# 294coder/Dif-PAN

Measured on AMD Instinct MI355X. Metric: fused megapixels/sec at T=1000, WV3 64x64x8 tiles, higher is better.
Workload: dtype f32-class (f16x2 split); 1 GPU; WV3 pansharpening, batch 64 of 64x64x8 tiles per GPU, T=1000 DDPM p_sample, fp32; tiles_per_gpu=64, tiles_total=64, T=1000, model_evaluations=1000, sampler=ddpm, parallelism=tile-shard x1, launches_per_denoising_step=132

## Files before the change

dif-pan_amd/csrc/conv_variants.h:

```cpp
#pragma once
#include "ddif_plan.h"
#include "kernels_conv.h"

namespace ddif {
namespace {

template <int KS, int S, int U, int CK, int PRO, int VEC, int EPI = 0>
ConvVariant variant_for_cfg(int cfg) {
    ConvVariant v;
    switch (cfg) {
        case 0: v.fn = conv_mfma_kernel<KS, S, U, 8, 16, CK, 4, 1, 1, 1, PRO, VEC, EPI>; v.smem = conv_smem_bytes<KS, S, U, 8, 16, CK, 1, PRO>(); v.th = 8; v.tw = 16; v.nt = 32; break;
        case 2: v.fn = conv_mfma_kernel<KS, S, U, 8, 8, CK, 2, 2, 1, 1, PRO, VEC, EPI>; v.smem = conv_smem_bytes<KS, S, U, 8, 8, CK, 2, PRO>(); v.th = 8; v.tw = 8; v.nt = 64; break;
        default: break;
    }
    if constexpr (KS == 1 && VEC == 1) {
        switch (cfg) {
            case 1: v.fn = conv_mfma_kernel<KS, S, U, 8, 16, CK, 4, 1, 1, 2, PRO, VEC, EPI>; v.smem = conv_smem_bytes<KS, S, U, 8, 16, CK, 2, PRO>(); v.th = 8; v.tw = 16; v.nt = 64; break;
            case 3: v.fn = conv_mfma_kernel<KS, S, U, 8, 16, CK, 4, 1, 1, 4, PRO, VEC, EPI>; v.smem = conv_smem_bytes<KS, S, U, 8, 16, CK, 4, PRO>(); v.th = 8; v.tw = 16; v.nt = 128; break;
            case 4: v.fn = conv_mfma_kernel<KS, S, U, 8, 8, CK, 2, 2, 1, 2, PRO, VEC, EPI>; v.smem = conv_smem_bytes<KS, S, U, 8, 8, CK, 4, PRO>(); v.th = 8; v.tw = 8; v.nt = 128; break;
            default: break;
        }
        if constexpr (CK == 32) {
            switch (cfg) {
                case 12: v.fn = conv_mfma_kernel<KS, S, U, 8, 16, CK, 4, 1, 1, 1, PRO, VEC, EPI, 0, 1>; v.smem = conv_smem_bytes<KS, S, U, 8, 16, CK, 1, PRO, 4, 1>(); v.th = 8; v.tw = 16; v.nt = 32; v.x3 = true; break;
// ... 43 lines not shown
        switch (cfg) {
            case 28: v.fn = conv_mfma_kernel<KS, S, U, 8, 16, CK, 4, 1, 1, 1, PRO, VEC, EPI, 0, 3>; v.smem = conv_smem_bytes<KS, S, U, 8, 16, CK, 1, PRO, 4, 3>(); v.th = 8; v.tw = 16; v.nt = 32; v.x3 = v.f16 = true; break;
            case 29: v.fn = conv_mfma_kernel<KS, S, U, 8, 8, CK, 2, 2, 1, 1, PRO, VEC, EPI, 0, 3>; v.smem = conv_smem_bytes<KS, S, U, 8, 8, CK, 2, PRO, 4, 3>(); v.th = 8; v.tw = 8; v.nt = 64; v.x3 = v.f16 = true; break;
            default: break;
        }
    }
    if constexpr (KS == 3 && S == 1 && U == 0 && VEC == 1) {
        switch (cfg) {
            case 5: v.fn = conv_mfma_kernel<KS, S, U, 16, 16, CK, 8, 1, 1, 1, PRO, VEC, EPI>; v.smem = conv_smem_bytes<KS, S, U, 16, 16, CK, 1, PRO, 8>(); v.th = 16; v.tw = 16; v.nt = 32; v.nthr = 512; break;
            case 6: v.fn = conv_mfma_kernel<KS, S, U, 16, 16, CK, 8, 1, 1, 2, PRO, VEC, EPI>; v.smem = conv_smem_bytes<KS, S, U, 16, 16, CK, 2, PRO, 8>(); v.th = 16; v.tw = 16; v.nt = 64; v.nthr = 512; break;
            default: break;
        }
    }
    return v;
}
template <int KS, int S, int U, int CK, int PRO, int VEC>
ConvVariant variant_small_tiles(int cfg) {
    return (cfg >= 2) ? variant_for_cfg<KS, S, U, CK, PRO, VEC>(cfg) : ConvVariant();
}
}
}
```

dif-pan_amd/csrc/ddif_capi.cpp:

```cpp
#include "ddif_plan.h"

struct ddif_net {
    ddif::Net n;
};
struct ddif_plan {
    ddif::Plan p;
};

namespace ddif {
extern int g_debug_grid_cap;
}

struct DeviceScope {
    int prev = -1;
    bool ok = true;
    explicit DeviceScope(int dev) {
        if (hipGetDevice(&prev) != hipSuccess) prev = -1;
        if (prev != dev) ok = hipSetDevice(dev) == hipSuccess;
    }
    ~DeviceScope() {
        int cur = -1;
        if (prev >= 0 && hipGetDevice(&cur) == hipSuccess && cur != prev) (void)hipSetDevice(prev);
    }
};
#define DDIF_PLAN_ENTER(plan, what)                                                                                   \
    if (!(plan)) return ddif::fail(DDIF_ERR_INVALID, what ": NULL plan");                                             \
    DeviceScope dscope__((plan)->p.net->device);                                                                      \
    if (!dscope__.ok) return ddif::fail(DDIF_ERR_HIP, what ": hipSetDevice(%d) failed", (plan)->p.net->device);      \
    if ((plan)->p.generation != (plan)->p.net->generation)                                                            \
        return ddif::fail(DDIF_ERR_STATE, what ": the network's weights were re-committed after this plan was built " \
                                               "(its launch program points into the old weight blob); create a new plan"); \
    if ((plan)->p.net->merged_stale && !(plan)->p.train_mode)                                                         \
        return ddif::fail(DDIF_ERR_STATE, what ": the weights were refreshed on the device for training (ddif_net_refresh), which leaves the "   \
                                               "inference-only merged FFN weights stale; load + commit the weights again before inference")

#define DDIF_GUARD_BEGIN try {
#define DDIF_GUARD_END                                                                    \
    }                                                                                     \
    catch (const std::exception& e) {                                                     \
        return ddif::fail(DDIF_ERR_INVALID, "unexpected C++ exception: %s", e.what());    \
    }                                                                                     \
    catch (...) {                                                                         \
        return ddif::fail(DDIF_ERR_INVALID, "unexpected C++ exception");                  \
    }

extern "C" {

int ddif_net_create(ddif_net_t* out, const ddif_net_cfg* cfg, int device) {
    DDIF_GUARD_BEGIN
// ... 389 lines not shown
```

dif-pan_amd/csrc/ddif_conv_k3.cpp:

```cpp
#include "conv_variants.h"

namespace ddif {

ConvVariant get_conv_variant_k3(int stride, int ups, int ck, int pro, int cfg, int vec) {
    ConvVariant v;
    const bool plain = stride == 1 && !ups;
    if (ck != 16) return v;
    if (vec == 2) {
        if (plain && pro == PRO_NONE) { v = variant_for_cfg<3, 1, 0, 16, PRO_NONE, 2>(cfg); v.name = "conv3x3_cat"; }
    } else if (!vec) {
        if (plain && pro == PRO_NONE) { v = variant_for_cfg<3, 1, 0, 16, PRO_NONE, 0>(cfg); v.name = "conv3x3_scalar"; }
    } else if (plain && pro == PRO_GN_SILU) { v = variant_for_cfg<3, 1, 0, 16, PRO_GN_SILU, 1>(cfg); v.name = "conv3x3_gn_silu"; }
    else if (plain && pro == PRO_NONE) { v = variant_for_cfg<3, 1, 0, 16, PRO_NONE, 1>(cfg); v.name = "conv3x3"; }
    else if (stride == 2 && !ups && pro == PRO_NONE) { v = variant_small_tiles<3, 2, 0, 16, PRO_NONE, 1>(cfg); v.name = "conv3x3_s2"; }
    else if (stride == 1 && ups && pro == PRO_NONE) { v = variant_for_cfg<3, 1, 1, 16, PRO_NONE, 1>(cfg); v.name = "conv3x3_up2"; }
    return v;
}

}
```

dif-pan_amd/csrc/ddif_net.cpp:

```cpp
#include "ddif_net.h"
#include <cstdint>
#include <tuple>
#include "kernels_refresh.h"

namespace ddif {

thread_local std::string g_err;

int fail(int code, const char* fmt, ...) {
    char buf[1024];
    va_list ap;
    va_start(ap, fmt);
    vsnprintf(buf, sizeof(buf), fmt, ap);
    va_end(ap);
    g_err = buf;
    return code;
}

static bool in_list(const int32_t* a, int n, int v) {
    for (int i = 0; i < n; ++i)
        if (a[i] == v) return true;
    return false;
}

// ... 221 lines not shown
                                for (int pl = 0; pl < 2; ++pl) {
                                    const size_t fl = (((((size_t)nbi * n_chunks + ch) * taps + tap) * K16 + k16) * 2 + pl) * 256 + (size_t)(h * 32 + j) * 4;
                                    o[fl * 2 + t] = q[pl];
                                }
                            }
    return off;
}

size_t pack_conv_b1(Blob& b, size_t x3_off, int cout, int cin, int ks, int ck) {
    const size_t steps = (size_t)((((cout + 31) / 32 + 3) & ~3)) * ((cin + ck - 1) / ck) * (ks * ks) * (ck / 16);
    const size_t off = b.add(nullptr, steps * 256);
    for (size_t st = 0; st < steps; ++st) std::memcpy(b.v.data() + off + st * 256, b.v.data() + x3_off + st * 3 * 256, 256 * sizeof(float));
    return off;
}

}

int Net::commit(hipStream_t stream) {
    Blob b;
    struct PendConv { std::string name; size_t w_off; long bias_off; int cin, cout, ks, ck, n_chunks; long x3_off = -1; long f16_off = -1; long b1_off = -1; };
    std::vector<PendConv> pend;
    std::map<std::string, size_t> vec_off;
    std::string missing;
    recipes.clear();
    auto rec_pack = [&](int kind, const std::string& s0, const std::string& s1, size_t off, int cout, int cin0, int cin1, int ks, int ck, int n_chunks) {
        Recipe r;
        r.kind = kind;
        r.src0 = s0;
        r.src1 = s1;
        r.dst_off = off;
        r.cout = cout;
        r.cin0 = cin0;
        r.cin1 = cin1;
        r.ks = ks;
        r.ck = ck;
// ... 107 lines not shown
                    for (int nb = 0; nb < co / 32; ++nb)
                        for (int ln = 0; ln < 64; ++ln)
                            for (int sx = 0; sx < 16; ++sx)
                                r[((size_t)nb * 64 + ln) * 16 + sx] = wx->v[(size_t)(32 * nb + (ln & 31)) * 32 + 8 * (sx >> 2) + 4 * (ln >> 5) + (sx & 3)];
                    vec_off[L.p + ".cond_inj.x_conv.xf"] = b.add(r.data(), r.size());
                }
            }
        }
    }
    for (auto& L : mid) {
        add_slot(L.p + ".res_block");
        add_resblock(L.p + ".res_block");
        if (L.attn) add_attn(L.p + ".attn");
    }
    for (auto& L : ups) {
        if (L.kind == L_UP) { add_conv(L.p + ".conv", true); continue; }
        add_slot(L.p + ".res_block");
        add_resblock(L.p + ".res_block");
        if (L.attn) add_attn(L.p + ".attn");
        const std::string ci = L.p + ".cond_inj";
        add_vec(ci + ".prenorm_x.weight");
        add_vec(ci + ".prenorm_x.bias");
        add_dw(ci + ".q.0.weight");
        add_conv(ci + ".q.1", true);
        add_dw(ci + ".kv.0.weight");
        add_conv(ci + ".kv.1", true);
        const HostTensor *wo = need(ci + ".attn_out.weight"), *bo = need(ci + ".attn_out.bias");
        const HostTensor* wr = get(ci + ".attn_res.weight");
        const HostTensor* br = get(ci + ".attn_res.bias");
        if (wo) {
            vec_off[ci + ".attn_out.weight"] = b.add(wo->v.data(), wo->v.size());
// ... 121 lines not shown
        blob = nullptr;
    }
    blob_floats = b.v.size() + 64;
    DDIF_HIPCHK(hipMalloc((void**)&blob, blob_floats * sizeof(float)));
    DDIF_HIPCHK(hipMemcpy(blob, b.v.data(), b.v.size() * sizeof(float), hipMemcpyHostToDevice));
    (void)stream;

    conv.clear();
    vec.clear();
    for (auto& p : pend) {
        PackedConv pc;
        pc.w = blob + p.w_off;
        pc.w_x3 = p.x3_off >= 0 ? blob + p.x3_off : nullptr;
        pc.w_f16 = p.f16_off >= 0 ? blob + p.f16_off : nullptr;
        pc.w_b1 = p.b1_off >= 0 ? blob + p.b1_off : nullptr;
        pc.bias = p.bias_off >= 0 ? blob + p.bias_off : nullptr;
        pc.cin = p.cin;
        pc.cout = p.cout;
        pc.ks = p.ks;
        pc.ck = p.ck;
        pc.n_chunks = p.n_chunks;
        conv[p.name] = pc;
    }
    vec_absmax.clear();
    for (auto& kv : vec_off) {
        vec[kv.first] = blob + kv.second;
        float m = 0.f;
        if (const HostTensor* t = get(kv.first))
            for (float x : t->v) m = std::fabs(x) > m || std::isnan(x) ? (std::isnan(x) ? INFINITY : std::fabs(x)) : m;
        vec_absmax[blob + kv.second] = m;
// ... 173 lines not shown
```

dif-pan_amd/csrc/ddif_net.h:

```cpp
#pragma once
#include <mutex>
#include <cmath>
#include <cstdarg>
#include <cstdint>
#include <cstdio>
#include <cstring>
#include <functional>
#include <map>
#include <memory>
#include <string>
#include <vector>

#include "../../include/ddif.h"
#include "../../include/ddif_testops.h"
#include "ddif_dev.h"

namespace ddif {

extern thread_local std::string g_err;
int fail(int code, const char* fmt, ...);

#define DDIF_HIPCHK(x)                                                                                      \
    do {                                                                                                    \
        hipError_t e__ = (x);                                                                               \
// ... 6 lines not shown

enum LayerKind { L_STEM, L_ENC, L_DOWN, L_MID, L_DEC, L_UP };

struct Layer {
    LayerKind kind;
    int cin = 0, cout = 0, cx = 0, cskip = 0;
    bool attn = false;
    std::string p;
};

struct PackedConv {
    const float* w = nullptr;
    const float* w_x3 = nullptr;
    const float* w_f16 = nullptr;
    const float* w_b1 = nullptr;
    const float* bias = nullptr;
    int cin = 0, cout = 0, ks = 1, ck = 32, n_chunks = 0;
};

struct HostTensor {
    std::vector<float> v;
    std::vector<int64_t> shape;
};

struct Net {
    ddif_net_cfg cfg{};
    int device = 0;
    std::vector<Layer> downs, mid, ups;
    int final_in = 0;
    std::map<std::string, HostTensor> host;
// ... 59 lines not shown
```

dif-pan_amd/csrc/ddif_plan.cpp:

```cpp
#include "ddif_plan.h"
#include <algorithm>
#include "kernels_conv.h"
#include "kernels_misc.h"
#include "attn_args.h"
#include "kernels_lafuse.h"

namespace ddif {

ConvVariant get_conv_variant(int ks, int stride, int ups, int ck, int pro, int cfg, int vec, int epi, int math) {
    if (cfg == 20 || cfg == 21)
        return (stride == 1 && !ups && vec == 1) ? get_lr_variant(ks, cfg == 20 ? 2 : 4, pro, epi, (math == MATH_F16X2 && pro == PRO_COLSM) ? MATH_BF16X3 : math) : ConvVariant();
    if (ks == 1) return get_conv_variant_k1(stride, ups, ck, pro, cfg, vec, epi);
    if (ks == 3) return epi ? get_conv_variant_k3e(stride, ups, ck, pro, cfg, vec, epi) : get_conv_variant_k3(stride, ups, ck, pro, cfg, vec);
    return ConvVariant();
}

static int num_cus();
static int x3_enabled() {
    static const int x3 = [] { const char* e = getenv("DDIF_X3"); return e ? atoi(e) : 1; }();
    return x3;
}
static int f16_enabled() {
    static const int f16 = [] { const char* e = getenv("DDIF_F16"); return e ? atoi(e) : 1; }();
    return f16;
}
int g_math_mode = [] { const char* e = getenv("DDIF_MATH"); return (e && std::strcmp(e, "bf16") == 0) ? 1 : 0; }();
int g_f16_raw = [] { const char* e = getenv("DDIF_F16_RAW"); return e ? (atoi(e) != 0) : 1; }();
static int lr_rows_enabled() {
    static const int v = [] { const char* e = getenv("DDIF_LR_ROWS"); return e ? atoi(e) : 1; }();
    return v;
}
static int lafuse_enabled() {
    static const int v = [] { const char* e = getenv("DDIF_LAFUSE"); return e ? atoi(e) : 1; }();
    return v;
}
static int xcd_mask() {
    static const int v = [] { const char* e = getenv("DDIF_XCD"); return e ? atoi(e) : 15; }();
    return v;
}
static int la8_enabled() {
    static const int v = [] { const char* e = getenv("DDIF_LA8"); return e ? atoi(e) : 1; }();
    return v;
}
static int xf_enabled() {
// ... 236 lines not shown
        return fail(DDIF_ERR_INVALID, "%s: a tensor of this batch reaches 4 GiB (32-bit offsets); split the batch", s.name);
    bool f16ok = f16_enabled() && !train_mode && pc.w_f16 && !s.w_override && !s.exact;
    const bool raw_in = !(s.pro == PRO_GN || s.pro == PRO_GN_SILU || s.pro == PRO_GN_DW);
    if (raw_in && !f16_raw) f16ok = false;
    if (f16ok && (s.pro == PRO_GN || s.pro == PRO_GN_SILU)) {
        auto ig = net->vec_absmax.find(s.gamma), ib = net->vec_absmax.find(s.beta);
        const double n = (double)(c0 + c1) * Hin * Win;
        f16ok = ig != net->vec_absmax.end() && ib != net->vec_absmax.end() && std::sqrt(n) * ig->second + ib->second < DDIF_F16_AMAX;
    }
    const bool b1ok = math_mode == 1 && !train_mode && pc.w_b1 && !s.w_override && !s.exact;
    const bool f16ok0 = f16ok;
    if (b1ok) f16ok = false;
    int math = b1ok ? MATH_BF16X1 : (f16ok ? MATH_F16X2 : MATH_BF16X3);
    int cfg = pick_cfg(pc.ks, pc.ck, s.pro, vec, s.stride, s.ups, Hout, Wout, pc.cout, B, c0 + c1, c1 ? c0 : c0 + c1, true, s.exact, f16ok, b1ok);
    const int epi = (s.film ? EPI_FILM : 0) | (s.res ? EPI_RES : 0) | (pc.cout % 4 != 0 ? EPI_SOUT : 0) | (s.silu ? EPI_SILU : 0) | (s.cso_mx ? EPI_COLST : 0);
    if (s.cso_mx && ((cfg != 20 && cfg != 21) || Hout > (cfg == 20 ? 8 : 16)))
        return fail(DDIF_ERR_INVALID, "%s: column statistics epilogue needs the low-resolution kernel and H <= 16", s.name);
    static const bool wres_env = [] { const char* e = getenv("DDIF_WRES"); return !e || atoi(e) != 0; }();
    if (cfg == 27 && wres_env && c0 == 32 && c1 == 0 && pc.cout <= 32 && pc.ck == 16 && pc.n_chunks == 2 && !s.w_override && s.w_bstride == 0 &&
        get_conv_variant(pc.ks, s.stride, s.ups, pc.ck, s.pro, 37, vec, epi, math).fn)
        cfg = 37;
    ConvVariant var = get_conv_variant(pc.ks, s.stride, s.ups, pc.ck, s.pro, cfg, vec, epi, math);
    if (!var.fn && (cfg == 20 || cfg == 21)) {
        cfg = pick_cfg(pc.ks, pc.ck, s.pro, vec, s.stride, s.ups, Hout, Wout, pc.cout, B, c0 + c1, c1 ? c0 : c0 + c1, false, false, f16ok, b1ok);
        var = get_conv_variant(pc.ks, s.stride, s.ups, pc.ck, s.pro, cfg, vec, epi);
    }
    if (!var.fn && b1ok) {
        f16ok = f16ok0;
        math = f16ok ? MATH_F16X2 : MATH_BF16X3;
        cfg = pick_cfg(pc.ks, pc.ck, s.pro, vec, s.stride, s.ups, Hout, Wout, pc.cout, B, c0 + c1, c1 ? c0 : c0 + c1, true, s.exact, f16ok, false);
        var = get_conv_variant(pc.ks, s.stride, s.ups, pc.ck, s.pro, cfg, vec, epi, math);
        if (!var.fn && (cfg == 20 || cfg == 21)) {
            cfg = pick_cfg(pc.ks, pc.ck, s.pro, vec, s.stride, s.ups, Hout, Wout, pc.cout, B, c0 + c1, c1 ? c0 : c0 + c1, false, false, f16ok, false);
            var = get_conv_variant(pc.ks, s.stride, s.ups, pc.ck, s.pro, cfg, vec, epi);
        }
    }
    if (!var.fn) return fail(DDIF_ERR_INVALID, "%s: no kernel variant (ks=%d stride=%d ups=%d ck=%d pro=%d cfg=%d vec=%d epi=%d)", s.name, pc.ks, s.stride, s.ups, pc.ck, s.pro, cfg, vec, epi);
// ... 27 lines not shown
        use(s.cso_mx);
        use(s.cso_sm);
    }
    if (int e = alloc_tensor(out, pc.cout, Hout, Wout, &prog == &step)) return e;
    if (xf) {
        if (int e = alloc_tensor(&s.xf->out, s.xf->pc->cout, Hout, Wout, true)) return e;
    }
    ConvArgs a{};
    a.in0 = s.in0.p;
    a.in1 = s.in1.p;
    a.c0 = c0;
    a.c1 = c1;
    a.B = B;
    a.Hin = Hin;
    a.Win = Win;
    a.Hout = Hout;
    a.Wout = Wout;
    a.Cout = pc.cout;
    a.w = s.w_override ? s.w_override : (var.b1 ? pc.w_b1 : (var.f16 ? pc.w_f16 : (var.x3 ? pc.w_x3 : pc.w)));
    if (var.x3 && !s.w_override && !a.w) return fail(DDIF_ERR_STATE, "%s: split-operand variant without split weights", s.name);
    a.w_bstride = s.w_bstride;
    a.cs_mx = s.cs_mx;
    a.cs_sm = s.cs_sm;
    a.dw_w = s.dw_w;
    a.out_xn = s.out_xn;
    a.cso_mx = s.cso_mx;
    a.cso_sm = s.cso_sm;
    if (s.pro == PRO_GN_DW && (!s.dw_w || c0 + c1 > 256)) return fail(DDIF_ERR_INVALID, "%s: depthwise staging needs weights and <= 256 channels", s.name);
    if (s.pro == PRO_COLSM && (!s.cs_mx || !s.cs_sm || c0 % pc.ck != 0)) return fail(DDIF_ERR_INVALID, "%s: column-softmax prologue needs statistics and c0 %% %d == 0", s.name, pc.ck);
    a.n_chunks = var.wr ? 1 : pc.n_chunks;
    a.bias = (s.use_bias && pc.bias) ? pc.bias : zeros;
    a.tbias = zeros;
    a.st0 = s.in0.st;
    a.np0 = s.in0.np;
    a.st1 = s.in1.st;
    a.np1 = s.in1.np;
    a.gamma = s.gamma;
    a.beta = s.beta;
    a.res = s.res;
    a.film = s.film;
    a.out = out->p;
    a.tiles_x = (Wout + var.tw - 1) / var.tw;
    a.tiles_y = (Hout + var.th - 1) / var.th;
    const int gy = (pc.cout + var.nt - 1) / var.nt;
    const bool st_halves = !var.lr && var.th == 16 && var.tw == 16 && var.nthr == 512;
    a.st_halves = st_halves ? 1 : 0;
    a.tiles_y8 = (Hout + 7) / 8;
    const int np_out = st_halves ? a.tiles_x * a.tiles_y8 : a.tiles_x * a.tiles_y;
    if (s.stats) {
        out->np = np_out * gy;
        if (int e = dalloc(&out->st, (size_t)B * out->np * 2)) return e;
        a.st_out = out->st;
    }
    a.n_ct = gy;
    if (xf) {
        if (gy != 1 || !s.stats) return fail(DDIF_ERR_STATE, "%s: x_conv fold needs one cout tile and output statistics", s.name);
        s.xf->out.np = np_out;
        if (int e = dalloc(&s.xf->out.st, (size_t)B * s.xf->out.np * 2)) return e;
        a.xf_w = s.xf->w;
        a.xf_b = s.xf->pc->bias;
        a.xf_film = s.xf->film;
        a.xf_out = s.xf->out.p;
// ... 31 lines not shown
        const ConvVariant vs = get_conv_variant(pc.ks, s.stride, s.ups, pc.ck, s.pro, cfg, vec, EPI_SAMP, math);
        if (vs.fn && vs.smem == var.smem) {
            fn_samp = vs.fn;
            if (var.smem + 8192 > 64 * 1024)
                DDIF_HIPCHK(hipFuncSetAttribute(reinterpret_cast<const void*>(fn_samp), hipFuncAttributeMaxDynamicSharedMemorySize, (int)(var.smem + 8192)));
            final_fused = true;
        }
    }
    const float* lms_p = lms.p;
    const bool dyn = s.dyn_input;
    const bool self_c = net->cfg.self_condition != 0;
    const int tb_off = s.tb_off;
    static const bool dump = getenv("DDIF_DUMP_PLAN") != nullptr;
    if (dump)
        fprintf(stderr, "[ddif plan] %-34s %-24s ks=%d s=%d u=%d  %3d+%3d -> %3d  @%3dx%-3d pro=%d epi=%d cfg=%d items=%ld grid=%u smem=%zu  in@%p out@%p\n", s.name, var.name, pc.ks, s.stride,
                s.ups, c0, c1, pc.cout, Hout, Wout, s.pro, epi, cfg, nwork, grid.x, smem, (const void*)s.in0.p, (const void*)out->p);
    Op op;
    op.name = var.name;
    {
        char lb[160];
        snprintf(lb, sizeof lb, "%s %dx%d %d+%d->%d @%dx%d cfg%d", s.name, pc.ks, pc.ks, c0, c1, pc.cout, Hout, Wout, cfg);
        op.label = lb;
    }
    op.flop = 2.0 * B * Hout * Wout * (double)pc.cout * (c0 + c1) * pc.ks * pc.ks;
    op.bytes = 4.0 * B * ((double)Hin * Win * (c0 + c1) + (double)Hout * Wout * pc.cout);
    if (xf) {
        op.label += " + x_conv+FiLM";
        op.flop += 2.0 * B * Hout * Wout * 32.0 * s.xf->pc->cout;
        op.bytes += 4.0 * B * (double)Hout * Wout * 3.0 * s.xf->pc->cout;
    }
    op.cls = (Hout * Wout <= 256) ? 2 : (pc.ks == 3 ? 0 : 1);
    op.mfma_w = var.b1 ? 1 : (var.f16 ? 3 : (var.x3 ? 6 : 16));
    op.timed = op.cls == 0;
    if (pc.ks == 3 && &prog == &step) {
        ++n_conv3;
        if (var.x3) ++n_conv3_x3;
        if (var.f16) ++n_conv3_f16;
        if (var.b1) ++n_conv3_b1;
    }
// ... 1527 lines not shown
```

dif-pan_amd/csrc/kernels_conv.h:

```cpp
#pragma once
#include "ddif_dev.h"
#include "sampler_dev.h"

namespace ddif {

struct ConvArgs {
    const float* in0;
    const float* in1;
    int c0, c1;
    int B, Hin, Win;
    int Hout, Wout, Cout;
    const float* w;
    int n_chunks;
    const float* bias;
    const float* tbias;
    int tbias_stride;
    const int* step_ptr;
    int tb_rowstride;
    const double* st0;
    int np0;
    const double* st1;
    int np1;
    const float* gamma;
    const float* beta;
// ... 28 lines not shown
    int xf_cout;
    int st_halves;
    int tiles_y8;
};

template <int F>
struct StageKind {
    static constexpr bool LAST = (F & 1) != 0;
    static constexpr bool TAIL = (F & 2) != 0;
};

enum { EPI_FILM = 1, EPI_SOUT = 2, EPI_RES = 4, EPI_SILU = 8, EPI_TBS = 16, EPI_COLST = 32, EPI_SAMP = 64, EPI_XF1 = 128, EPI_XF2 = 256 };
template <int KS, int STRIDE, int UPS, int TH, int TW, int CK, int WM, int WN, int MB, int NB, int PRO, int VEC, int EPI = 0, int ABL = 0, int MATH = 0>
__global__ __launch_bounds__(64 * WM * WN) void conv_mfma_kernel(ConvArgs a) {
    constexpr int NW = WM * WN, NTHR = 64 * NW;
    constexpr int PAD = KS / 2;
    constexpr int IH = (TH - 1) * STRIDE + KS, IW = (TW - 1) * STRIDE + KS;
    constexpr bool X3 = MATH >= 1;
    constexpr bool F16 = MATH == 3 || MATH == 5;
    constexpr bool WR = MATH == 5;
    constexpr bool B1 = MATH == 4;
    constexpr int NPL = F16 ? 2 : (B1 ? 1 : 3);
    constexpr bool WSB = MATH == 2;
    constexpr int NWB = (WSB || WR) ? 1 : 2;
    constexpr int PS = CK / 2;
    constexpr int LDA = X3 ? NPL * PS + 4 : CK + 4;
    constexpr int LDH = CK + 4;
    constexpr int TAPS = KS * KS;
    constexpr int K8 = CK / 8;
    constexpr int K16 = CK / 16;
    constexpr int C4 = CK / 4;
    constexpr int NF = X3 ? TAPS * K16 : TAPS * K8;
    constexpr int RP = (X3 && KS == 3 && STRIDE == 1) ? (WR ? (64 - (IW * LDA) % 64) % 64 : (NPL == 2 ? 24 : (NPL == 1 ? 40 : 8))) : 0;
    constexpr int LDR = IW * LDA + RP;
    constexpr int ABUF = IH * LDR;
    constexpr bool DWM = (PRO == PRO_GN_DW);
    constexpr bool GNP = (PRO == PRO_GN || PRO == PRO_GN_SILU || PRO == PRO_GN_DW);
    constexpr bool FILM = (EPI & EPI_FILM) != 0, SOUT = (EPI & EPI_SOUT) != 0, RES = (EPI & EPI_RES) != 0, SILU = (EPI & EPI_SILU) != 0, TBS = (EPI & EPI_TBS) != 0;
    constexpr bool SAMP = (EPI & EPI_SAMP) != 0;
    constexpr int NBX = (EPI & EPI_XF1) ? 1 : ((EPI & EPI_XF2) ? 2 : 0);
    constexpr bool XF = NBX > 0;
    static_assert(!SAMP || (!SOUT && !RES && !FILM), "sampler epilogue: the plain vector epilogue of the final conv");
    static_assert(!XF || (MB == 1 && NB == 1 && WN == 1 && !SOUT && !SAMP && !FILM && !SILU && PRO != PRO_GN_DW), "x_conv + FiLM fold: one wave holds all 32 couts of its pixels");
// ... 7 lines not shown
    constexpr int NITEMS = (LH * LW * C4 + NTHR - 1) / NTHR;
    constexpr int WCHUNK = X3 ? NF * NPL * 256 : NF * 256;
    constexpr int WBUF = NB * WN * WCHUNK;
    constexpr int WITEMS = WR ? 0 : (WBUF / 4 + NTHR - 1) / NTHR;
    constexpr int WITEMS_A = WITEMS ? WITEMS : 1;
    constexpr int WRI = WR ? (WBUF / 4 + NTHR - 1) / NTHR : 1;
    constexpr int DUMMY = DWM ? CK : (X3 ? NPL * PS : CK);
    static_assert(NW == 4 || NW == 8, "4 or 8 wavefronts per workgroup");
    static_assert(!X3 || (CK % 16 == 0 && (VEC == 1 || (VEC == 2 && F16 && PRO == PRO_NONE))), "split-operand paths: 16-channel slabs, float4 staging (per-thread source select: the stem on f16x2)");
    static_assert(TH * TW == 32 * MB * WM, "pixel tile must match the wave layout");
    static_assert(CK % 8 == 0 && NTHR % C4 == 0, "chunk size");
    static_assert(NITEMS <= 32, "valid mask is 32 bits");
    static_assert(!F16 || PRO != PRO_COLSM, "f16x2: the column-softmax prologue stays on bf16x3 / fp32 (probabilities far below 2^-7)");
    static_assert(RP == 0 || !DWM, "row pad: 3x3 tiles only");
    static_assert(!WR || (KS == 3 && STRIDE == 1 && !UPS && CK == 32 && TW == 16 && !DWM), "resident weights: plain 3x3 convs with one 32-channel stage");

    dd_touch_kernargs<sizeof(ConvArgs)>();
    DDIF_DYN_SMEM(smem);
    float* As = reinterpret_cast<float*>(smem);
    float* Ws = As + 2 * ABUF;
    double* red = reinterpret_cast<double*>(smem + (size_t)(2 * ABUF + NWB * WBUF) * sizeof(float));
    float* Hs = reinterpret_cast<float*>(smem + (size_t)(2 * ABUF + NWB * WBUF) * sizeof(float) + 4 * NW * sizeof(double));
    float* DWs = Hs + HBUF;
    [[maybe_unused]] double* redx = reinterpret_cast<double*>(DWs + DWMAX);
    float* GBs = DWs + DWMAX + (XF ? 8 * NW : 0);
    float* BTs = GBs + (GNP ? 2 * a.n_chunks * CK : 0);
    [[maybe_unused]] float* BXs = BTs + a.n_ct * (32 * NB * WN);

    const int tid = threadIdx.x, lane = tid & 63;
#ifdef DDIF_EMU
    const int wave = tid >> 6;
    [[maybe_unused]] const long long t_entry = 0;
#else
    const int wave = __builtin_amdgcn_readfirstlane(tid >> 6);
    [[maybe_unused]] const long long t_entry = (ABL & 16) ? (long long)__builtin_amdgcn_s_memtime() : 0;
#endif
    const int wm = wave / WN, wn = wave % WN;
    const int h = lane >> 5, j = lane & 31;
    const int tiles = a.tiles_x * a.tiles_y;
    const int ntiles = a.B * tiles;
    const int nwork = ntiles * a.n_ct;
    int w0, w1;
    wg_work_range(nwork, &w0, &w1, a.xcd);
    if (w0 >= w1) return;
    const int Hc = UPS ? a.Hin * 2 : a.Hin, Wc = UPS ? a.Win * 2 : a.Win;
    const int Ctot = a.c0 + a.c1;
    const int GBN = a.n_chunks * CK;
    const int c4 = tid % C4;
    const int stepv = a.step_ptr ? *a.step_ptr : 0;
    const float* tbrow = a.tbias;
    [[maybe_unused]] SamplerRun s_run{};
    [[maybe_unused]] int s_k = 0;
    [[maybe_unused]] float s_c0 = 0.f, s_c1 = 0.f, s_c2 = 0.f, s_c3 = 0.f, s_c4 = 0.f;
    [[maybe_unused]] const float* s_noise = nullptr;
    if constexpr (SAMP) {
        s_run = *a.s_run;
        s_k = *a.step_ptr;
        s_c0 = s_run.tab[0][s_k];
        s_c1 = s_run.tab[1][s_k];
        s_c2 = s_run.tab[2][s_k];
// ... 2 lines not shown
            s_c4 = s_run.tab[4][s_k];
        }
        s_noise = s_run.noise ? s_run.noise + (size_t)s_k * ((size_t)a.B * a.Cout * a.Hout * a.Wout) : nullptr;
        if (blockIdx.x == 0 && tid == 0) *a.s_step_next = s_k + 1;
    }

    int abase[MB], e_my[MB], e_mx[MB];
    unsigned e_off[MB], e_foff[MB];
    [[maybe_unused]] unsigned e_xoff[MB], e_xfoff[MB];
#pragma unroll
    for (int mb = 0; mb < MB; ++mb) {
        const int m = (wm * MB + mb) * 32 + j;
        abase[mb] = (m / TW) * STRIDE * LDR + (m % TW) * STRIDE * LDA + 4 * h;
        e_my[mb] = m / TW;
        e_mx[mb] = m % TW;
        e_off[mb] = (unsigned)(((e_my[mb] * a.Wout + e_mx[mb]) * a.Cout + 4 * h) * 4);
        e_foff[mb] = (unsigned)(((e_my[mb] * a.Wout + e_mx[mb]) * 2 * a.Cout + 4 * h) * 4);
        if constexpr (XF) {
            e_xoff[mb] = (unsigned)(((e_my[mb] * a.Wout + e_mx[mb]) * (32 * NBX) + 4 * h) * 4);
            e_xfoff[mb] = (unsigned)(((e_my[mb] * a.Wout + e_mx[mb]) * 2 * (32 * NBX) + 4 * h) * 4);
        }
    }
    [[maybe_unused]] float xw[XF ? NBX : 1][16];
    if constexpr (XF) {
#pragma unroll
        for (int nx = 0; nx < NBX; ++nx)
#pragma unroll
            for (int q = 0; q < 4; ++q) {
                const float4 t = *reinterpret_cast<const float4*>(a.xf_w + ((size_t)(nx * 64 + lane) * 16 + 4 * q));
                xw[nx][4 * q + 0] = t.x;
                xw[nx][4 * q + 1] = t.y;
// ... 58 lines not shown
    Pos L = locate(w0);
    int l_ch = 0;
    [[maybe_unused]] int l_sp[(VEC == 1) ? 1 : NITEMS];
    [[maybe_unused]] unsigned l_o0[NITEMS], l_o1[NITEMS];
    unsigned l_cso[PRO == PRO_COLSM ? NITEMS : 1];
    unsigned l_ok = 0;
    auto item_geometry = [&]() {
        const int iy0 = L.oy0 * STRIDE - LPAD, ix0 = L.ox0 * STRIDE - LPAD;
        l_ok = 0;
#pragma unroll
        for (int it = 0; it < NITEMS; ++it) {
            const int iy = iy0 + a_py[it], ix = ix0 + a_px[it];
            const bool ok = (iy >= 0) & (iy < Hc) & (ix >= 0) & (ix < Wc);
            l_ok |= (ok ? 1u : 0u) << it;
            const int iyc = iy < 0 ? 0 : (iy >= Hc ? Hc - 1 : iy), ixc = ix < 0 ? 0 : (ix >= Wc ? Wc - 1 : ix);
            const int sp = (L.b * a.Hin + (UPS ? (iyc >> 1) : iyc)) * a.Win + (UPS ? (ixc >> 1) : ixc);
            if constexpr (VEC == 1) {
                l_o0[it] = (unsigned)sp * (unsigned)(a.c0 * 4);
                if (a.c1) l_o1[it] = (unsigned)sp * (unsigned)(a.c1 * 4);
            } else {
                l_sp[it] = sp;
            }
            if (PRO == PRO_COLSM) l_cso[it] = (unsigned)(L.b * a.Win + ixc) * (unsigned)(a.c0 * 4);
        }
        l_ok &= a_in;
    };

    struct StageRegs {
        float4 sv[NITEMS], wv[WITEMS_A];
        float4 mxv[PRO == PRO_COLSM ? NITEMS : 1], smv[PRO == PRO_COLSM ? NITEMS : 1];
        unsigned ok;
// ... 265 lines not shown
        if ((ABL & 16) && a.dbg && tid == 0 && dbg_n < 126) a.dbg[blockIdx.x * 128 + dbg_n++] = (long long)__builtin_amdgcn_s_memtime();
#endif
    };
#ifndef DDIF_EMU
    if ((ABL & 16) && a.dbg && tid == 0) a.dbg[blockIdx.x * 128 + dbg_n++] = t_entry;
#endif
    f32x16 acc[MB][NB];
    const int nflat = (w1 - w0) * a.n_chunks;

    auto stage = [&](auto kind, const int cur, StageRegs& Rn, StageRegs& Rf) {
        constexpr bool LAST = decltype(kind)::LAST, TAIL = decltype(kind)::TAIL;
        stamp();
        const float* Ac = As + cur * ABUF;
        const Pos Cp = bufpos[cur];
        const int c_ch = bufch[cur];
        const int nbg0 = (Cp.ct * WN + wn) * NB;
        float4 e_t[(LAST && TBS) ? NB : 1][4];
        float4 e_res[(LAST && RES) ? MB : 1][(LAST && RES) ? NB : 1][4];
        float4 e_fs[(LAST && FILM) ? MB : 1][(LAST && FILM) ? NB : 1][4], e_fh[(LAST && FILM) ? MB : 1][(LAST && FILM) ? NB : 1][4];
        [[maybe_unused]] float4 e_xi[(LAST && SAMP) ? MB : 1][(LAST && SAMP) ? NB : 1][4], e_xl[(LAST && SAMP) ? MB : 1][(LAST && SAMP) ? NB : 1][4];
        [[maybe_unused]] float4 e_xs[(LAST && XF) ? NBX : 1][4], e_xh[(LAST && XF) ? NBX : 1][4];
        [[maybe_unused]] unsigned e_pxo = 0;
        bool full = true;
        unsigned e_po[MB], e_pf[MB];
        bool e_pok[MB];
        size_t tile_el = 0;
        if constexpr (LAST) {
            full = (Cp.oy0 + TH <= a.Hout) & (Cp.ox0 + TW <= a.Wout);
            const size_t tile_pix = (size_t)((Cp.b * a.Hout + Cp.oy0) * a.Wout + Cp.ox0);
            tile_el = tile_pix * a.Cout + nbg0 * 32;
#pragma unroll
            for (int mb = 0; mb < MB; ++mb) {
                e_pok[mb] = full || ((Cp.oy0 + e_my[mb] < a.Hout) & (Cp.ox0 + e_mx[mb] < a.Wout));
                e_po[mb] = e_pok[mb] ? e_off[mb] : (unsigned)(16 * h);
                e_pf[mb] = e_pok[mb] ? e_foff[mb] : (unsigned)(16 * h);
            }
            if constexpr (!SOUT) {
                const int nbl = nbg0 * 32 < a.Cout ? nbg0 * 32 : 0;
                [[maybe_unused]] const char* tb = reinterpret_cast<const char*>(tbrow + (size_t)Cp.b * a.tbias_stride + nbl);
                [[maybe_unused]] const char* rbase = reinterpret_cast<const char*>(a.res + tile_pix * a.Cout + nbl);
                [[maybe_unused]] const char* fbase = reinterpret_cast<const char*>(a.film + tile_pix * 2 * a.Cout + nbl);
                [[maybe_unused]] const char* xibase = reinterpret_cast<const char*>(a.s_img + tile_pix * a.Cout + nbl);
                [[maybe_unused]] const char* xlbase = reinterpret_cast<const char*>(a.s_lms + tile_pix * a.Cout + nbl);
#pragma unroll
// ... 35 lines not shown
        if (c_ch == 0) {
#pragma unroll
            for (int mb = 0; mb < MB; ++mb)
#pragma unroll
                for (int nb = 0; nb < NB; ++nb)
#pragma unroll
                    for (int r = 0; r < 16; ++r) acc[mb][nb][r] = 0.f;
        }
        if constexpr (ILV && !TAIL) fs_begin(Rn);
        const float* Wc = Ws + ((WSB || WR) ? 0 : cur) * WBUF + (wn * NB) * WCHUNK + h * 128 + j * 4;
        if constexpr (X3) {
            constexpr int FB = (MB * NB >= 2) ? 1 : 2;
            float4 xa[FB][MB][NPL], wb[FB][NB][NPL];
            auto load_frags3 = [&](int f, int slot) {
                const int tap = WR ? f % TAPS : f / K16, k16 = WR ? f / TAPS : f % K16;
                const int aoff = (tap / KS) * LDR + (tap % KS) * LDA + k16 * 8;
#pragma unroll
                for (int q = 0; q < NPL; ++q) {
#pragma unroll
                    for (int mb = 0; mb < MB; ++mb)
                        xa[slot][mb][q] = (ABL & 128) ? make_float4(1.f, 2.f, 3.f, (float)(f + q)) : *reinterpret_cast<const float4*>(&Ac[abase[mb] + aoff + q * PS]);
#pragma unroll
                    for (int nb = 0; nb < NB; ++nb)
                        wb[slot][nb][q] = (ABL & 128) ? make_float4(4.f, 3.f, 2.f, (float)(f - q)) : *reinterpret_cast<const float4*>(&Wc[nb * WCHUNK + (f * NPL + q) * 256]);
                }
            };
            if (FB == 2) load_frags3(0, 0);
#pragma unroll
            for (int tap = 0; tap < NF; ++tap) {
                if (FB == 2) {
                    if (tap + 1 < NF) load_frags3(tap + 1, (tap + 1) & 1);
// ... 285 lines not shown
    if (DWM) {
#pragma unroll
        for (int k = 0; k < DWI; ++k) {
            const int i = tid + k * NTHR;
            if (i < 9 * Ctot) DWs[i] = t_dw[k];
        }
    }
    if (GNP) {
        gn_reduce_partials(gp, a.st0, a.np0, a.st1, a.np1, R0.pos.b, (double)Ctot * a.Hin * a.Win, &mean, &rstd);
        gn_b = R0.pos.b;
    }
    __syncthreads();
    stamp();
    finish_stage(R0, 0);
    {
        const int nbt = a.n_ct * (32 * NB * WN);
#pragma unroll
        for (int k = 0; k < TBL; ++k) {
            const int i = tid + k * NTHR;
            if (i < nbt) BTs[i] = t_bias[k] + t_tb[k];
        }
        for (int i = tid + TBL * NTHR; i < nbt; i += NTHR) {
            const int c = i < a.Cout ? i : a.Cout - 1;
            BTs[i] = a.bias[c] + (TBS ? 0.f : tbrow[c]);
        }
        if constexpr (XF) {
            if (tid < 32 * NBX) BXs[tid] = a.xf_b[tid];
        }
    }
    __syncthreads();
    stamp();
// ... 15 lines not shown
    if (nflat & 1) stage(StageKind<3>{}, 0, R1, R0);
    __syncthreads();
    flush_stats();
    stamp();
    if constexpr (RANGE) {
        if (a.range_flag && !(r_max < 65520.f)) *a.range_flag = 1;
    }
}


template <int KS, int STRIDE, int UPS, int TH, int TW, int CK, int NBT, int PRO = 0, int NW = 4, int MATH = 0>
constexpr size_t conv_smem_bytes() {
    constexpr int IH = (TH - 1) * STRIDE + KS, IW = (TW - 1) * STRIDE + KS;
    constexpr size_t dw = PRO == PRO_GN_DW ? (size_t)((TH + 2) * (TW + 2) * (CK + 4) + 9 * 256) : 0;
    constexpr int npl = (MATH == 3 || MATH == 5) ? 2 : (MATH == 4 ? 1 : 3);
    constexpr int lda = MATH >= 1 ? npl * CK / 2 + 4 : CK + 4, wchunk = MATH >= 1 ? KS * KS * (CK / 16) * npl * 256 : KS * KS * (CK / 8) * 256;
    constexpr int rp = (MATH >= 1 && KS == 3 && STRIDE == 1) ? (MATH == 5 ? (64 - (IW * lda) % 64) % 64 : (npl == 2 ? 24 : (npl == 1 ? 40 : 8))) : 0;
    return (size_t)(2 * IH * (IW * lda + rp) + ((MATH == 2 || MATH == 5) ? 1 : 2) * NBT * wchunk + dw) * sizeof(float) + 4 * NW * sizeof(double);
}
inline size_t conv_smem_extra(int pro, int n_chunks, int ck, int cout_pad, int xf_cout = 0) {
    return ((pro == PRO_GN || pro == PRO_GN_SILU || pro == PRO_GN_DW) ? (size_t)2 * n_chunks * ck : 0) * sizeof(float) + (size_t)cout_pad * sizeof(float) +
           (xf_cout ? (size_t)xf_cout * sizeof(float) + 32 * sizeof(double) : 0);
}

}
```

Baseline: 0.07824 MP/s.

## Fold nearest-upsample into 3x3 conv as four 2x2 polyphase convs

Nearest-2x upsample followed by a 3x3 conv is rewritten as four phase-specific 2x2 convolutions on the low-resolution input. The weights are pre-summed on the host at commit time into a 4*cout f16x2 pack. The kernel gains a polyphase mode that selects the phase from the output-channel tile, offsets the input window, and writes interleaved outputs. This cuts the MACs from 9 to 4 taps per output and avoids reading the upsampled input. In exchange it adds a new kernel variant, a larger grid, and a separate weight pack that goes stale after weight refresh.

```diff
diff --git a/dif-pan_amd/csrc/conv_variants.h b/dif-pan_amd/csrc/conv_variants.h
--- a/dif-pan_amd/csrc/conv_variants.h
+++ b/dif-pan_amd/csrc/conv_variants.h
@@ -81,6 +81,16 @@
     }
     return v;
 }
+inline ConvVariant variant_up_poly(int cfg) {
+    ConvVariant v;
+    switch (cfg) {
+        case 27: v.fn = conv_mfma_kernel<3, 1, 2, 16, 16, 16, 8, 1, 1, 2, PRO_NONE, 1, 0, 0, 3>; v.smem = conv_smem_bytes<3, 1, 2, 16, 16, 16, 2, PRO_NONE, 8, 3>(); v.th = 16; v.tw = 16; v.nt = 64; v.nthr = 512; v.x3 = v.f16 = true; break;
+        case 28: v.fn = conv_mfma_kernel<3, 1, 2, 8, 16, 16, 4, 1, 1, 2, PRO_NONE, 1, 0, 0, 3>; v.smem = conv_smem_bytes<3, 1, 2, 8, 16, 16, 2, PRO_NONE, 4, 3>(); v.th = 8; v.tw = 16; v.nt = 64; v.x3 = v.f16 = true; break;
+        case 29: v.fn = conv_mfma_kernel<3, 1, 2, 8, 8, 16, 2, 2, 1, 1, PRO_NONE, 1, 0, 0, 3>; v.smem = conv_smem_bytes<3, 1, 2, 8, 8, 16, 2, PRO_NONE, 4, 3>(); v.th = 8; v.tw = 8; v.nt = 64; v.x3 = v.f16 = true; break;
+        default: break;
+    }
+    return v;
+}
 template <int KS, int S, int U, int CK, int PRO, int VEC>
 ConvVariant variant_small_tiles(int cfg) {
     return (cfg >= 2) ? variant_for_cfg<KS, S, U, CK, PRO, VEC>(cfg) : ConvVariant();
diff --git a/dif-pan_amd/csrc/ddif_capi.cpp b/dif-pan_amd/csrc/ddif_capi.cpp
--- a/dif-pan_amd/csrc/ddif_capi.cpp
+++ b/dif-pan_amd/csrc/ddif_capi.cpp
@@ -32,7 +32,7 @@
                                                "(its launch program points into the old weight blob); create a new plan"); \
     if ((plan)->p.net->merged_stale && !(plan)->p.train_mode)                                                         \
         return ddif::fail(DDIF_ERR_STATE, what ": the weights were refreshed on the device for training (ddif_net_refresh), which leaves the "   \
-                                               "inference-only merged FFN weights stale; load + commit the weights again before inference")
+                                               "inference-only packs (merged FFN weights, f16x2 planes, polyphase Upsample folds) stale; load + commit the weights again before inference")
 
 #define DDIF_GUARD_BEGIN try {
 #define DDIF_GUARD_END                                                                    \
diff --git a/dif-pan_amd/csrc/ddif_conv_k3.cpp b/dif-pan_amd/csrc/ddif_conv_k3.cpp
--- a/dif-pan_amd/csrc/ddif_conv_k3.cpp
+++ b/dif-pan_amd/csrc/ddif_conv_k3.cpp
@@ -13,7 +13,8 @@
     } else if (plain && pro == PRO_GN_SILU) { v = variant_for_cfg<3, 1, 0, 16, PRO_GN_SILU, 1>(cfg); v.name = "conv3x3_gn_silu"; }
     else if (plain && pro == PRO_NONE) { v = variant_for_cfg<3, 1, 0, 16, PRO_NONE, 1>(cfg); v.name = "conv3x3"; }
     else if (stride == 2 && !ups && pro == PRO_NONE) { v = variant_small_tiles<3, 2, 0, 16, PRO_NONE, 1>(cfg); v.name = "conv3x3_s2"; }
-    else if (stride == 1 && ups && pro == PRO_NONE) { v = variant_for_cfg<3, 1, 1, 16, PRO_NONE, 1>(cfg); v.name = "conv3x3_up2"; }
+    else if (stride == 1 && ups == 1 && pro == PRO_NONE) { v = variant_for_cfg<3, 1, 1, 16, PRO_NONE, 1>(cfg); v.name = "conv3x3_up2"; }
+    else if (stride == 1 && ups == 2 && pro == PRO_NONE) { v = variant_up_poly(cfg); v.name = "conv3x3_up2_poly"; }
     return v;
 }
 
diff --git a/dif-pan_amd/csrc/ddif_net.cpp b/dif-pan_amd/csrc/ddif_net.cpp
--- a/dif-pan_amd/csrc/ddif_net.cpp
+++ b/dif-pan_amd/csrc/ddif_net.cpp
@@ -259,11 +259,27 @@
     return off;
 }
 
+std::vector<float> fold_up_poly(const float* w, int cout, int cin) {
+    static const int lo[2][2] = {{0, 1}, {0, 2}}, hi[2][2] = {{0, 2}, {1, 2}};
+    std::vector<float> f((size_t)4 * cout * cin * 4);
+    for (int ph = 0; ph < 4; ++ph)
+        for (int o = 0; o < cout; ++o)
+            for (int i = 0; i < cin; ++i)
+                for (int t = 0; t < 4; ++t) {
+                    const int py = ph >> 1, px = ph & 1, ty = t >> 1, tx = t & 1;
+                    double acc = 0.0;
+                    for (int ky = lo[py][ty]; ky <= hi[py][ty]; ++ky)
+                        for (int kx = lo[px][tx]; kx <= hi[px][tx]; ++kx) acc += (double)w[((size_t)o * cin + i) * 9 + ky * 3 + kx];
+                    f[(((size_t)ph * cout + o) * cin + i) * 4 + t] = (float)acc;
+                }
+    return f;
+}
+
 }
 
 int Net::commit(hipStream_t stream) {
     Blob b;
-    struct PendConv { std::string name; size_t w_off; long bias_off; int cin, cout, ks, ck, n_chunks; long x3_off = -1; long f16_off = -1; long b1_off = -1; };
+    struct PendConv { std::string name; size_t w_off; long bias_off; int cin, cout, ks, ck, n_chunks; long x3_off = -1; long f16_off = -1; long b1_off = -1; long up4_off = -1; };
     std::vector<PendConv> pend;
     std::map<std::string, size_t> vec_off;
     std::string missing;
@@ -401,7 +417,17 @@
         if (L.attn) add_attn(L.p + ".attn");
     }
     for (auto& L : ups) {
-        if (L.kind == L_UP) { add_conv(L.p + ".conv", true); continue; }
+        if (L.kind == L_UP) {
+            add_conv(L.p + ".conv", true);
+            const HostTensor* w = get(L.p + ".conv.weight");
+            if (w && w->shape.size() == 4 && w->shape[2] == 3 && w->shape[3] == 3 && !pend.empty() && pend.back().name == L.p + ".conv") {
+                const int co = (int)w->shape[0], cin = (int)w->shape[1];
+                const std::vector<float> f = fold_up_poly(w->v.data(), co, cin);
+                const size_t off = pack_conv_f16(b, f.data(), 4 * co, cin, 2, 16);
+                pend.back().up4_off = off == (size_t)-1 ? -1 : (long)off;
+            }
+            continue;
+        }
         add_slot(L.p + ".res_block");
         add_resblock(L.p + ".res_block");
         if (L.attn) add_attn(L.p + ".attn");
@@ -553,6 +579,7 @@
         pc.w_x3 = p.x3_off >= 0 ? blob + p.x3_off : nullptr;
         pc.w_f16 = p.f16_off >= 0 ? blob + p.f16_off : nullptr;
         pc.w_b1 = p.b1_off >= 0 ? blob + p.b1_off : nullptr;
+        pc.w_up4 = p.up4_off >= 0 ? blob + p.up4_off : nullptr;
         pc.bias = p.bias_off >= 0 ? blob + p.bias_off : nullptr;
         pc.cin = p.cin;
         pc.cout = p.cout;
diff --git a/dif-pan_amd/csrc/ddif_net.h b/dif-pan_amd/csrc/ddif_net.h
--- a/dif-pan_amd/csrc/ddif_net.h
+++ b/dif-pan_amd/csrc/ddif_net.h
@@ -44,6 +44,7 @@
     const float* w_x3 = nullptr;
     const float* w_f16 = nullptr;
     const float* w_b1 = nullptr;
+    const float* w_up4 = nullptr;
     const float* bias = nullptr;
     int cin = 0, cout = 0, ks = 1, ck = 32, n_chunks = 0;
 };
diff --git a/dif-pan_amd/csrc/ddif_plan.cpp b/dif-pan_amd/csrc/ddif_plan.cpp
--- a/dif-pan_amd/csrc/ddif_plan.cpp
+++ b/dif-pan_amd/csrc/ddif_plan.cpp
@@ -28,6 +28,10 @@
 int g_f16_raw = [] { const char* e = getenv("DDIF_F16_RAW"); return e ? (atoi(e) != 0) : 1; }();
 static int lr_rows_enabled() {
     static const int v = [] { const char* e = getenv("DDIF_LR_ROWS"); return e ? atoi(e) : 1; }();
+    return v;
+}
+static int up_poly_enabled() {
+    static const int v = [] { const char* e = getenv("DDIF_UP_POLY"); return e ? atoi(e) : 1; }();
     return v;
 }
 static int lafuse_enabled() {
@@ -294,13 +298,19 @@
     int math = b1ok ? MATH_BF16X1 : (f16ok ? MATH_F16X2 : MATH_BF16X3);
     int cfg = pick_cfg(pc.ks, pc.ck, s.pro, vec, s.stride, s.ups, Hout, Wout, pc.cout, B, c0 + c1, c1 ? c0 : c0 + c1, true, s.exact, f16ok, b1ok);
     const int epi = (s.film ? EPI_FILM : 0) | (s.res ? EPI_RES : 0) | (pc.cout % 4 != 0 ? EPI_SOUT : 0) | (s.silu ? EPI_SILU : 0) | (s.cso_mx ? EPI_COLST : 0);
+    const bool poly = s.ups && up_poly_enabled() && x3_enabled() && f16ok && !b1ok && pc.w_up4 && pc.ks == 3 && pc.ck == 16 && vec == 1 && c1 == 0 && s.pro == PRO_NONE &&
+                      epi == 0 && s.tb_off < 0 && !s.samp && pc.cout % 32 == 0;
+    if (poly) cfg = Win >= 16 ? pick_cfg(3, 16, PRO_NONE, 1, 1, 0, Hin, Win, pc.cout, B, c0, c0, false, false, true, false) : 29;
+    const int ups_k = poly ? 2 : s.ups;
+    const int Hk = poly ? Hin : Hout, Wk = poly ? Win : Wout;
     if (s.cso_mx && ((cfg != 20 && cfg != 21) || Hout > (cfg == 20 ? 8 : 16)))
         return fail(DDIF_ERR_INVALID, "%s: column statistics epilogue needs the low-resolution kernel and H <= 16", s.name);
     static const bool wres_env = [] { const char* e = getenv("DDIF_WRES"); return !e || atoi(e) != 0; }();
     if (cfg == 27 && wres_env && c0 == 32 && c1 == 0 && pc.cout <= 32 && pc.ck == 16 && pc.n_chunks == 2 && !s.w_override && s.w_bstride == 0 &&
         get_conv_variant(pc.ks, s.stride, s.ups, pc.ck, s.pro, 37, vec, epi, math).fn)
         cfg = 37;
-    ConvVariant var = get_conv_variant(pc.ks, s.stride, s.ups, pc.ck, s.pro, cfg, vec, epi, math);
+    ConvVariant var = get_conv_variant(pc.ks, s.stride, ups_k, pc.ck, s.pro, cfg, vec, epi, math);
+    if (poly && !var.fn) return fail(DDIF_ERR_STATE, "%s: no polyphase Upsample variant for cfg %d", s.name, cfg);
     if (!var.fn && (cfg == 20 || cfg == 21)) {
         cfg = pick_cfg(pc.ks, pc.ck, s.pro, vec, s.stride, s.ups, Hout, Wout, pc.cout, B, c0 + c1, c1 ? c0 : c0 + c1, false, false, f16ok, b1ok);
         var = get_conv_variant(pc.ks, s.stride, s.ups, pc.ck, s.pro, cfg, vec, epi);
@@ -358,10 +368,10 @@
     a.B = B;
     a.Hin = Hin;
     a.Win = Win;
-    a.Hout = Hout;
-    a.Wout = Wout;
+    a.Hout = Hk;
+    a.Wout = Wk;
     a.Cout = pc.cout;
-    a.w = s.w_override ? s.w_override : (var.b1 ? pc.w_b1 : (var.f16 ? pc.w_f16 : (var.x3 ? pc.w_x3 : pc.w)));
+    a.w = s.w_override ? s.w_override : (var.b1 ? pc.w_b1 : (poly ? pc.w_up4 : (var.f16 ? pc.w_f16 : (var.x3 ? pc.w_x3 : pc.w))));
     if (var.x3 && !s.w_override && !a.w) return fail(DDIF_ERR_STATE, "%s: split-operand variant without split weights", s.name);
     a.w_bstride = s.w_bstride;
     a.cs_mx = s.cs_mx;
@@ -384,12 +394,12 @@
     a.res = s.res;
     a.film = s.film;
     a.out = out->p;
-    a.tiles_x = (Wout + var.tw - 1) / var.tw;
-    a.tiles_y = (Hout + var.th - 1) / var.th;
-    const int gy = (pc.cout + var.nt - 1) / var.nt;
+    a.tiles_x = (Wk + var.tw - 1) / var.tw;
+    a.tiles_y = (Hk + var.th - 1) / var.th;
+    const int gy = (poly ? 4 : 1) * ((pc.cout + var.nt - 1) / var.nt);
     const bool st_halves = !var.lr && var.th == 16 && var.tw == 16 && var.nthr == 512;
     a.st_halves = st_halves ? 1 : 0;
-    a.tiles_y8 = (Hout + 7) / 8;
+    a.tiles_y8 = (Hk + 7) / 8;
     const int np_out = st_halves ? a.tiles_x * a.tiles_y8 : a.tiles_x * a.tiles_y;
     if (s.stats) {
         out->np = np_out * gy;
@@ -451,7 +461,7 @@
     static const bool dump = getenv("DDIF_DUMP_PLAN") != nullptr;
     if (dump)
         fprintf(stderr, "[ddif plan] %-34s %-24s ks=%d s=%d u=%d  %3d+%3d -> %3d  @%3dx%-3d pro=%d epi=%d cfg=%d items=%ld grid=%u smem=%zu  in@%p out@%p\n", s.name, var.name, pc.ks, s.stride,
-                s.ups, c0, c1, pc.cout, Hout, Wout, s.pro, epi, cfg, nwork, grid.x, smem, (const void*)s.in0.p, (const void*)out->p);
+                ups_k, c0, c1, pc.cout, Hout, Wout, s.pro, epi, cfg, nwork, grid.x, smem, (const void*)s.in0.p, (const void*)out->p);
     Op op;
     op.name = var.name;
     {
@@ -459,7 +469,7 @@
         snprintf(lb, sizeof lb, "%s %dx%d %d+%d->%d @%dx%d cfg%d", s.name, pc.ks, pc.ks, c0, c1, pc.cout, Hout, Wout, cfg);
         op.label = lb;
     }
-    op.flop = 2.0 * B * Hout * Wout * (double)pc.cout * (c0 + c1) * pc.ks * pc.ks;
+    op.flop = 2.0 * B * Hout * Wout * (double)pc.cout * (c0 + c1) * (poly ? 4 : pc.ks * pc.ks);
     op.bytes = 4.0 * B * ((double)Hin * Win * (c0 + c1) + (double)Hout * Wout * pc.cout);
     if (xf) {
         op.label += " + x_conv+FiLM";
diff --git a/dif-pan_amd/csrc/kernels_conv.h b/dif-pan_amd/csrc/kernels_conv.h
--- a/dif-pan_amd/csrc/kernels_conv.h
+++ b/dif-pan_amd/csrc/kernels_conv.h
@@ -66,6 +66,7 @@
 template <int KS, int STRIDE, int UPS, int TH, int TW, int CK, int WM, int WN, int MB, int NB, int PRO, int VEC, int EPI = 0, int ABL = 0, int MATH = 0>
 __global__ __launch_bounds__(64 * WM * WN) void conv_mfma_kernel(ConvArgs a) {
     constexpr int NW = WM * WN, NTHR = 64 * NW;
+    constexpr bool PP = UPS == 2;
     constexpr int PAD = KS / 2;
     constexpr int IH = (TH - 1) * STRIDE + KS, IW = (TW - 1) * STRIDE + KS;
     constexpr bool X3 = MATH >= 1;
@@ -78,7 +79,7 @@
     constexpr int PS = CK / 2;
     constexpr int LDA = X3 ? NPL * PS + 4 : CK + 4;
     constexpr int LDH = CK + 4;
-    constexpr int TAPS = KS * KS;
+    constexpr int TAPS = PP ? 4 : KS * KS;
     constexpr int K8 = CK / 8;
     constexpr int K16 = CK / 16;
     constexpr int C4 = CK / 4;
@@ -116,6 +117,7 @@
     static_assert(!F16 || PRO != PRO_COLSM, "f16x2: the column-softmax prologue stays on bf16x3 / fp32 (probabilities far below 2^-7)");
     static_assert(RP == 0 || !DWM, "row pad: 3x3 tiles only");
     static_assert(!WR || (KS == 3 && STRIDE == 1 && !UPS && CK == 32 && TW == 16 && !DWM), "resident weights: plain 3x3 convs with one 32-channel stage");
+    static_assert(!PP || (KS == 3 && STRIDE == 1 && F16 && !WR && PRO == PRO_NONE && VEC == 1 && EPI == 0), "polyphase Upsample conv: f16x2, raw input, plain epilogue");
 
     dd_touch_kernargs<sizeof(ConvArgs)>();
     DDIF_DYN_SMEM(smem);
@@ -145,7 +147,7 @@
     int w0, w1;
     wg_work_range(nwork, &w0, &w1, a.xcd);
     if (w0 >= w1) return;
-    const int Hc = UPS ? a.Hin * 2 : a.Hin, Wc = UPS ? a.Win * 2 : a.Win;
+    const int Hc = UPS == 1 ? a.Hin * 2 : a.Hin, Wc = UPS == 1 ? a.Win * 2 : a.Win;
     const int Ctot = a.c0 + a.c1;
     const int GBN = a.n_chunks * CK;
     const int c4 = tid % C4;
@@ -178,7 +180,8 @@
         abase[mb] = (m / TW) * STRIDE * LDR + (m % TW) * STRIDE * LDA + 4 * h;
         e_my[mb] = m / TW;
         e_mx[mb] = m % TW;
-        e_off[mb] = (unsigned)(((e_my[mb] * a.Wout + e_mx[mb]) * a.Cout + 4 * h) * 4);
+        e_off[mb] = PP ? (unsigned)(((2 * e_my[mb] * (2 * a.Wout) + 2 * e_mx[mb]) * a.Cout + 4 * h) * 4)
+                       : (unsigned)(((e_my[mb] * a.Wout + e_mx[mb]) * a.Cout + 4 * h) * 4);
         e_foff[mb] = (unsigned)(((e_my[mb] * a.Wout + e_mx[mb]) * 2 * a.Cout + 4 * h) * 4);
         if constexpr (XF) {
             e_xoff[mb] = (unsigned)(((e_my[mb] * a.Wout + e_mx[mb]) * (32 * NBX) + 4 * h) * 4);
@@ -267,7 +270,7 @@
             const bool ok = (iy >= 0) & (iy < Hc) & (ix >= 0) & (ix < Wc);
             l_ok |= (ok ? 1u : 0u) << it;
             const int iyc = iy < 0 ? 0 : (iy >= Hc ? Hc - 1 : iy), ixc = ix < 0 ? 0 : (ix >= Wc ? Wc - 1 : ix);
-            const int sp = (L.b * a.Hin + (UPS ? (iyc >> 1) : iyc)) * a.Win + (UPS ? (ixc >> 1) : ixc);
+            const int sp = (L.b * a.Hin + (UPS == 1 ? (iyc >> 1) : iyc)) * a.Win + (UPS == 1 ? (ixc >> 1) : ixc);
             if constexpr (VEC == 1) {
                 l_o0[it] = (unsigned)sp * (unsigned)(a.c0 * 4);
                 if (a.c1) l_o1[it] = (unsigned)sp * (unsigned)(a.c1 * 4);
@@ -563,7 +566,11 @@
         const float* Ac = As + cur * ABUF;
         const Pos Cp = bufpos[cur];
         const int c_ch = bufch[cur];
-        const int nbg0 = (Cp.ct * WN + wn) * NB;
+        [[maybe_unused]] const int c_nctp = PP ? (a.n_ct >> 2) : a.n_ct;
+        [[maybe_unused]] const int c_ph = PP ? Cp.ct / c_nctp : 0;
+        const int c_ctl = PP ? Cp.ct - c_ph * c_nctp : Cp.ct;
+        [[maybe_unused]] const int c_pofs = PP ? (c_ph >> 1) * LDR + (c_ph & 1) * LDA : 0;
+        const int nbg0 = (c_ctl * WN + wn) * NB;
         float4 e_t[(LAST && TBS) ? NB : 1][4];
         float4 e_res[(LAST && RES) ? MB : 1][(LAST && RES) ? NB : 1][4];
         float4 e_fs[(LAST && FILM) ? MB : 1][(LAST && FILM) ? NB : 1][4], e_fh[(LAST && FILM) ? MB : 1][(LAST && FILM) ? NB : 1][4];
@@ -576,7 +583,8 @@
         size_t tile_el = 0;
         if constexpr (LAST) {
             full = (Cp.oy0 + TH <= a.Hout) & (Cp.ox0 + TW <= a.Wout);
-            const size_t tile_pix = (size_t)((Cp.b * a.Hout + Cp.oy0) * a.Wout + Cp.ox0);
+            const size_t tile_pix = PP ? (size_t)((Cp.b * 2 * a.Hout + 2 * Cp.oy0 + (c_ph >> 1)) * 2 * a.Wout + 2 * Cp.ox0 + (c_ph & 1))
+                                       : (size_t)((Cp.b * a.Hout + Cp.oy0) * a.Wout + Cp.ox0);
             tile_el = tile_pix * a.Cout + nbg0 * 32;
 #pragma unroll
             for (int mb = 0; mb < MB; ++mb) {
@@ -642,7 +650,7 @@
             float4 xa[FB][MB][NPL], wb[FB][NB][NPL];
             auto load_frags3 = [&](int f, int slot) {
                 const int tap = WR ? f % TAPS : f / K16, k16 = WR ? f / TAPS : f % K16;
-                const int aoff = (tap / KS) * LDR + (tap % KS) * LDA + k16 * 8;
+                const int aoff = PP ? c_pofs + (tap / 2) * LDR + (tap % 2) * LDA + k16 * 8 : (tap / KS) * LDR + (tap % KS) * LDA + k16 * 8;
 #pragma unroll
                 for (int q = 0; q < NPL; ++q) {
 #pragma unroll
@@ -958,7 +966,7 @@
     stamp();
     finish_stage(R0, 0);
     {
-        const int nbt = a.n_ct * (32 * NB * WN);
+        const int nbt = (PP ? a.n_ct >> 2 : a.n_ct) * (32 * NB * WN);
 #pragma unroll
         for (int k = 0; k < TBL; ++k) {
             const int i = tid + k * NTHR;
@@ -1004,7 +1012,8 @@
     constexpr int IH = (TH - 1) * STRIDE + KS, IW = (TW - 1) * STRIDE + KS;
     constexpr size_t dw = PRO == PRO_GN_DW ? (size_t)((TH + 2) * (TW + 2) * (CK + 4) + 9 * 256) : 0;
     constexpr int npl = (MATH == 3 || MATH == 5) ? 2 : (MATH == 4 ? 1 : 3);
-    constexpr int lda = MATH >= 1 ? npl * CK / 2 + 4 : CK + 4, wchunk = MATH >= 1 ? KS * KS * (CK / 16) * npl * 256 : KS * KS * (CK / 8) * 256;
+    constexpr int taps = UPS == 2 ? 4 : KS * KS;
+    constexpr int lda = MATH >= 1 ? npl * CK / 2 + 4 : CK + 4, wchunk = MATH >= 1 ? taps * (CK / 16) * npl * 256 : taps * (CK / 8) * 256;
     constexpr int rp = (MATH >= 1 && KS == 3 && STRIDE == 1) ? (MATH == 5 ? (64 - (IW * lda) % 64) % 64 : (npl == 2 ? 24 : (npl == 1 ? 40 : 8))) : 0;
     return (size_t)(2 * IH * (IW * lda + rp) + ((MATH == 2 || MATH == 5) ? 1 : 2) * NBT * wchunk + dw) * sizeof(float) + 4 * NW * sizeof(double);
 }
```

New measurement: 0.07904 MP/s, median of 6. 1.01x the previous value.
